# soldasim/BOSS.jl

Hardware: AMD Instinct MI355X
Metric: gp_posterior_updates_per_sec (+ acq_evals_per_sec), N=4096 d=8 fp64 (higher is better)
Workload: dtype f64; 1 GPU; d=8 synthetic blackbox, GaussianProcess(Matern52) surrogate, N=4096 fp64 posterior update + ExpectedImprovement over 8192 candidates per GPU (BASELINE.json configs[1]+[2]); N=4096, d=8, M_per_gpu=8192, kernel=matern52, parallelism=single GPU: no exchange

## Files before the change

### boss.jl_amd/csrc/bosship.hip

```cpp
#include "../../include/bosship.h"

#include <hip/hip_runtime.h>

#include <algorithm>
#include <cmath>
#include <cstdint>
#include <cstdio>
#include <cstdlib>
#include <atomic>
#include <chrono>
#include <cstring>
#include <functional>
#include <limits>
#include <map>
#include <mutex>
#include <string>
#include <thread>
#include <vector>

#include "gp_kernels.hpp"
#include "potrf.hpp"
#include "chain.hpp"
#include "small_calls.hpp"
#include "rider.hpp"
// ... 225 lines not shown
        HIPCHK(hipEventCreateWithFlags(&c->llg_join[i], hipEventDisableTiming));
    }
    c->lookahead = !(getenv("BOSS_NO_LOOKAHEAD") && atoi(getenv("BOSS_NO_LOOKAHEAD")));
    {
        auto set_nonzero = [](const char* name) {
            const char* v = getenv(name);
            return v && *v && std::strcmp(v, "0") != 0;
        };
        static const bool gate_off = set_nonzero("BOSS_NO_GATE") || set_nonzero("ROCPROF_COUNTER_COLLECTION") || getenv("ROCPROF_COUNTERS") ||
                                     getenv("ROCPROF_COUNTER_GROUPS") || set_nonzero("ROCPROF_ADVANCED_THREAD_TRACE") ||
                                     getenv("ROCPROF_ATT_PARAM_SERIALIZE_ALL") || getenv("ROCP_METRICS") || set_nonzero("AMD_SERIALIZE_KERNEL");
        if (!gate_off) {
            if (set_nonzero("BOSS_DEBUG_WATCH")) {
                unsigned long long* hp = nullptr;
                HIPCHK(hipHostMalloc((void**)&hp, SIG_WORDS * sizeof(unsigned long long), hipHostMallocMapped));
                std::memset(hp, 0, SIG_WORDS * sizeof(unsigned long long));
                HIPCHK(hipHostGetDevicePointer((void**)&c->sig_panel, hp, 0));
                c->sig_panel_host = hp;
#ifdef BOSS_DEBUG_WATCH_BUILD
                HIPCHK(hipMemcpyToSymbol(HIP_SYMBOL(boss::g_dbg), &c->sig_panel, sizeof(void*)));
#endif
                std::thread([hp]() {
                    unsigned long long last[SIG_WORDS] = {0};
                    for (;;) {
                        std::this_thread::sleep_for(std::chrono::milliseconds(500));
                        unsigned long long now[SIG_WORDS];
                        for (int i = 0; i < SIG_WORDS; ++i) now[i] = ((volatile unsigned long long*)hp)[i];
                        if (std::memcmp(now, last, sizeof now) == 0) continue;
                        std::memcpy(last, now, sizeof now);
                        std::fprintf(stderr, "[bosship watch] up %llu wdone %llu panel %llu crit %llu | gate %llu near %llu bulk %llu | strips",
                                     now[SIGW_UP], now[SIGW_WDONE], now[SIGW_PANEL], now[SIGW_CRIT], now[SIGW_GATE], now[SIGW_NEAR], now[SIGW_BULK]);
                        for (int q = 0; q < 8; ++q) std::fprintf(stderr, " %llu", now[SIGW_PROG + SIGW_PROG_STRIDE * q]);
                        std::fprintf(stderr, " | give-ups: first %llu n %llu last %llu; waits ended by mark %llu, by clock %llu", now[SIGW_DBG], now[SIGW_DBG + 1],
                                     now[SIGW_DBG + 2], now[SIGW_DBG + 4], now[SIGW_DBG + 5]);
                        std::fprintf(stderr, "\n");
                    }
                }).detach();
            } else {
                HIPCHK(hipMalloc((void**)&c->sig_panel, SIG_WORDS * sizeof(unsigned long long)));
                HIPCHK(hipMemset(c->sig_panel, 0, SIG_WORDS * sizeof(unsigned long long)));
            }
        }
        c->chain_ok = !gate_off && !set_nonzero("BOSS_NO_CHAIN") && !set_nonzero("HIP_LAUNCH_BLOCKING");
        c->test_drop_chain = set_nonzero("BOSS_TEST_DROP_CHAIN");
        if (c->chain_ok) {
            int* okw = nullptr;
            HIPCHK(hipMalloc((void**)&okw, 4 * sizeof(int)));
            HIPCHK(hipMemset(okw, 0, 4 * sizeof(int)));
            hipStream_t probed[4] = {c->own_stream, c->side_stream, c->chain_stream, c->strip_stream};
            for (int i = 0; i < 4; ++i)
                hipLaunchKernelGGL(chain_probe_wait_kernel, dim3(1), dim3(64), 0, probed[i], c->sig_panel + SIGW_NEAR + 1, 4ull, okw + i);
            int okh[4] = {0, 0, 0, 0};
            bool fine = hipDeviceSynchronize() == hipSuccess && hipMemcpy(okh, okw, sizeof okh, hipMemcpyDeviceToHost) == hipSuccess;
            (void)hipFree(okw);
            if (!(fine && okh[0] && okh[1] && okh[2] && okh[3])) c->chain_ok = false;
            if (getenv("BOSS_CHAIN_VERBOSE"))
                std::fprintf(stderr, "[bosship] resident chain: %s (main / side / chain / strip streams side by side: %d %d %d %d)\n",
                             c->chain_ok ? "on" : "off", okh[0], okh[1], okh[2], okh[3]);
        }
    }
    HIPCHK(hipHostMalloc(&c->pinned, PINNED_BYTES, hipHostMallocDefault));
    std::memset(c->pinned, 0, PINNED_UP_OFF);
    HIPCHK(hipFuncSetAttribute((const void*)potrf_diag_kernel, hipFuncAttributeMaxDynamicSharedMemorySize, DIAG_LDS_BYTES));
    HIPCHK(hipFuncSetAttribute((const void*)potrf_chain_kernel, hipFuncAttributeMaxDynamicSharedMemorySize, CHAIN_LDS_BYTES));
    HIPCHK(hipFuncSetAttribute((const void*)potrf_strips_kernel, hipFuncAttributeMaxDynamicSharedMemorySize, STRIPS_LDS_BYTES));
    {
        int cus = 0;
        if (hipDeviceGetAttribute(&cus, hipDeviceAttributeMultiprocessorCount, c->device) != hipSuccess) cus = 0;
        if (cus > 0) c->n_cus = cus;
    }
    HIPCHK(hipFuncSetAttribute((const void*)small_fit_kernel, hipFuncAttributeMaxDynamicSharedMemorySize, SMALL_LDS_BYTES));
    HIPCHK(hipFuncSetAttribute((const void*)small_llgrad_kernel, hipFuncAttributeMaxDynamicSharedMemorySize, SMALL_LLG_LDS_BYTES));
    HIPCHK(hipFuncSetAttribute((const void*)small_fit_batch_kernel, hipFuncAttributeMaxDynamicSharedMemorySize, SMALL_LDS_BYTES));
    HIPCHK(hipFuncSetAttribute((const void*)small_predict_grad_kernel<true>, hipFuncAttributeMaxDynamicSharedMemorySize, SPG_LDS_BYTES));
    HIPCHK(hipFuncSetAttribute((const void*)small_predict_grad_kernel<false>, hipFuncAttributeMaxDynamicSharedMemorySize, SPG_LDS_BYTES));
    HIPCHK(hipFuncSetAttribute((const void*)potrf_syrk_kernel<2, true>, hipFuncAttributeMaxDynamicSharedMemorySize, 96 * 1024));
    HIPCHK(hipFuncSetAttribute((const void*)rider_step_kernel, hipFuncAttributeMaxDynamicSharedMemorySize, 96 * 1024));
    HIPCHK(hipFuncSetAttribute((const void*)predict_kernel<PredG32>, hipFuncAttributeMaxDynamicSharedMemorySize,
                               PredictLds<PredG32>::BYTES));
    HIPCHK(hipFuncSetAttribute((const void*)prune_head_kernel<PredG32>, hipFuncAttributeMaxDynamicSharedMemorySize,
                               PredictLds<PredG32>::BYTES));
    HIPCHK(hipFuncSetAttribute((const void*)predict_kernel_set<PredG32>, hipFuncAttributeMaxDynamicSharedMemorySize,
                               PredictLds<PredG32>::BYTES));
    HIPCHK(hipFuncSetAttribute((const void*)grad_accum_kernel, hipFuncAttributeMaxDynamicSharedMemorySize, 150 * 1024));
    HIPCHK(hipFuncSetAttribute((const void*)winv_gemv_kernel<1>, hipFuncAttributeMaxDynamicSharedMemorySize, 150 * 1024));
    HIPCHK(hipFuncSetAttribute((const void*)winv_gemv_kernel<2>, hipFuncAttributeMaxDynamicSharedMemorySize, 150 * 1024));
    HIPCHK(hipFuncSetAttribute((const void*)winv_gemv_kernel<4>, hipFuncAttributeMaxDynamicSharedMemorySize, 150 * 1024));
    HIPCHK(hipFuncSetAttribute((const void*)winv_args_kernel<1>, hipFuncAttributeMaxDynamicSharedMemorySize, 150 * 1024));
    HIPCHK(hipFuncSetAttribute((const void*)winv_args_kernel<2>, hipFuncAttributeMaxDynamicSharedMemorySize, 150 * 1024));
    HIPCHK(hipFuncSetAttribute((const void*)winv_args_kernel<4>, hipFuncAttributeMaxDynamicSharedMemorySize, 150 * 1024));
    HIPCHK(hipFuncSetAttribute((const void*)winv_args_kernel<1, true>, hipFuncAttributeMaxDynamicSharedMemorySize, 150 * 1024));
    HIPCHK(hipFuncSetAttribute((const void*)few_back_finish_kernel<PredG32>, hipFuncAttributeMaxDynamicSharedMemorySize,
                               PredictLds<PredG32>::BYTES));
    HIPCHK(hipFuncSetAttribute((const void*)few_w_kernel<PredG32>, hipFuncAttributeMaxDynamicSharedMemorySize, PredictLds<PredG32>::BYTES));
    HIPCHK(hipFuncSetAttribute((const void*)few_finish_kernel<PredG32>, hipFuncAttributeMaxDynamicSharedMemorySize,
                               PredictLds<PredG32>::BYTES));
    HIPCHK(hipFuncSetAttribute((const void*)linvt_kernel<PredG32>, hipFuncAttributeMaxDynamicSharedMemorySize,
                               PredictLds<PredG32>::BYTES));
    HIPCHK(hipFuncSetAttribute((const void*)backsolve_kernel<PredG32>, hipFuncAttributeMaxDynamicSharedMemorySize,
                               PredictLds<PredG32>::BYTES));
    HIPCHK(hipFuncSetAttribute((const void*)backsolve_set_kernel<PredG32>, hipFuncAttributeMaxDynamicSharedMemorySize,
                               PredictLds<PredG32>::BYTES));
    HIPCHK(hipFuncSetAttribute((const void*)grad_accum_set_kernel, hipFuncAttributeMaxDynamicSharedMemorySize, 150 * 1024));
    HIPCHK(hipFuncSetAttribute((const void*)predict_kernel<PredG64>, hipFuncAttributeMaxDynamicSharedMemorySize,
                               PredictLds<PredG64>::BYTES));
    HIPCHK(hipFuncSetAttribute((const void*)predict_kernel<PredG32, true>, hipFuncAttributeMaxDynamicSharedMemorySize,
                               PredictLds<PredG32>::BYTES));
    HIPCHK(hipFuncSetAttribute((const void*)predict_kernel<PredG64, true>, hipFuncAttributeMaxDynamicSharedMemorySize,
                               PredictLds<PredG64>::BYTES));
    HIPCHK(hipFuncSetAttribute((const void*)ei_mc_grad_set_kernel, hipFuncAttributeMaxDynamicSharedMemorySize, MC_GRAD_MAX_LDS));
    HIPCHK(hipFuncSetAttribute((const void*)acqp_grad_set_kernel, hipFuncAttributeMaxDynamicSharedMemorySize, ACQP_GRAD_MAX_LDS));
    HIPCHK(hipFuncSetAttribute((const void*)mean_eval_kernel<true>, hipFuncAttributeMaxDynamicSharedMemorySize, MEAN_MAX_LDS));
    HIPCHK(hipFuncSetAttribute((const void*)kprog_llgrad_tile_kernel, hipFuncAttributeMaxDynamicSharedMemorySize, KPROG_GRAD_MAX_LDS));
    HIPCHK(hipFuncSetAttribute((const void*)kprog_grad_accum_kernel, hipFuncAttributeMaxDynamicSharedMemorySize, KPROG_GRAD_MAX_LDS));
    return BOSS_OK;
}

static int virtual_devices() {
    static const int v = getenv("BOSS_VIRTUAL_DEVICES") ? std::max(0, atoi(getenv("BOSS_VIRTUAL_DEVICES"))) : 0;
    return v;
}
static int visible_devices(int* nphys_out = nullptr) {
    int n = 0;
    if (hipGetDeviceCount(&n) != hipSuccess || n <= 0) return 0;
    if (nphys_out) *nphys_out = n;
    return virtual_devices() > 0 ? virtual_devices() : n;
}

static int get_ctx(int device, Ctx** out) {
    std::lock_guard<std::mutex> lk(g_ctx_mtx);
    auto it = g_ctx.find(device);
    if (it != g_ctx.end()) {
        *out = it->second;
        HIPCHK(hipSetDevice(it->second->device));
        return BOSS_OK;
    }
    int nphys = 0;
    const int n = visible_devices(&nphys);
    if (n <= 0) return fail(BOSS_E_NO_DEVICE, "no HIP device visible (bosship has no CPU fallback)");
    if (device < 0 || device >= n) return fail(BOSS_E_INVALID, "device index out of range");
    const int phys = device % nphys;
    HIPCHK(hipSetDevice(phys));
    Ctx* c = new Ctx();
    c->device = phys;
    c->logical = device;
    int rc = ctx_init(c);
    if (rc) {
        ctx_destroy(c);
        return rc;
    }
    g_ctx[device] = c;
    *out = c;
    return BOSS_OK;
}

static int ws_reserve(Workspace& w, size_t bytes) {
    if (w.bytes >= bytes) return BOSS_OK;
    if (w.p) (void)hipFree(w.p);
    w.p = nullptr;
    w.bytes = 0;
    HIPCHK(dev_malloc(&w.p, bytes));
    w.bytes = bytes;
    return BOSS_OK;
}

struct ProfScope {
// ... 20 lines not shown
        hipEvent_t e;
        (void)hipEventCreate(&e);
        return e;
    }
};

struct boss_gpset {
    Ctx* ctx = nullptr;
    std::atomic<int> refs{0};
    void* slab = nullptr;
    void* host_block = nullptr;
    size_t slab_bytes = 0, host_bytes = 0;
};
static bool slab_cache_on() {
    static const bool v = !(getenv("BOSS_SLAB_CACHE") && atoi(getenv("BOSS_SLAB_CACHE")) == 0) &&
                          !poison_alloc();
    return v;
}
static void gpset_release_storage(boss_gpset* st) {
    Ctx* c = st->ctx;
    void *slab = st->slab, *hb = st->host_block;
    if (c && slab_cache_on()) {
        std::lock_guard<std::mutex> lk(c->slab_mtx);
        if (slab && st->slab_bytes > c->slab_cache_bytes) {
            std::swap(slab, c->slab_cache);
            c->slab_cache_bytes = st->slab_bytes;
        }
        if (hb && st->host_bytes > c->hostblk_cache_bytes) {
            std::swap(hb, c->hostblk_cache);
            c->hostblk_cache_bytes = st->host_bytes;
        }
    }
    if (slab) (void)hipFree(slab);
    if (hb) (void)hipHostFree(hb);
    st->slab = st->host_block = nullptr;
}

struct boss_gp {
    Ctx* ctx = nullptr;
    boss_gpset* set = nullptr;
    int kernel = 0, d = 0, N = 0, Np = 0, nblk = 0, ld = 0;
    double *Xraw = nullptr, *Xsc = nullptr, *y = nullptr, *mean = nullptr, *A = nullptr;
    double *LT = nullptr, *DT2 = nullptr, *avec = nullptr;
    bool have_lt = false;
    double *inv16 = nullptr, *Dinv = nullptr, *Dinv2 = nullptr, *hyp = nullptr, *invlam = nullptr, *scal = nullptr;
    int* info = nullptr;
    unsigned char* discrete_dev = nullptr;
    std::vector<unsigned char> discrete;
    double amp2 = 0.0;
    bool has_mean = false, fitted = false, pending = false, have_dinv = false;
    bool dinv_used = false;
    bool dinv_used_prev = false;
    bool gated = false;
    bool chained = false;
    bool fell_back = false;
    int trail_used = -1;
    double* host_res = nullptr;
    double* host_res_dev = nullptr;
    bool par_in_args = false;
    unsigned long long res_seq = 0;
    bool res_polled = false;
    double* host_par = nullptr;
    hipEvent_t par_ev = nullptr;
    unsigned long long epoch = 0;
    unsigned long long factor_gen = 0, dinv0_gen = ~0ull;
    hipEvent_t dinv_ev = nullptr;
    bool dinv_pending = false;
    bool aug = false;
    int npts = 0, ldx = 0, nhead = 0;
    bool gibbs = false;
    double *lamX = nullptr, *ampX = nullptr, *noiseX = nullptr;
    bool kprog = false;
    bool kgrad = false;
    FitProg* kp = nullptr;
    double *Winv = nullptr, *Linv = nullptr;
    double* W2 = nullptr;
    int w2_np = 0;
    unsigned long long w2_gen = ~0ull;
    bool w2_used = false;
    bool have_winv = false;
    int few_calls = 0;
    int append_calls = 0;
    double* prune_a = nullptr;
    int prune_a_np = 0;
    unsigned long long prune_a_gen = ~0ull;
    int prune_skip = 0, prune_backoff = 0;
    int append_path = 0;
};

struct boss_cand {
    Ctx* ctx = nullptr;
    int d = 0, M = 0, Mp = 0;
    double* Craw = nullptr;
};

struct boss_track {
    Ctx* ctx = nullptr;
    boss_gp* gp = nullptr;
    int d = 0, M = 0, Mp = 0, tiles = 0, Ncap = 0, N = 0;
    unsigned long long epoch = 0;
    double *V = nullptr, *Csc = nullptr, *mu = nullptr, *var = nullptr, *mean = nullptr;
    bool has_mean = false;
    bool gibbs = false;
    double *Clam = nullptr, *Camp = nullptr;
    bool aug = false;
};

static inline int round_up(int x, int m) { return (x + m - 1) / m * m; }
struct SetBatch {
    int nb = 1;
    size_t sA = 0, sInv16 = 0, sDinv = 0, sDinv2 = 0, sW = 0, sX = 0;
    size_t sPar = 0;
};
struct MeanFold {
    const double* J = nullptr;
    size_t sJ = 0;
    int T = 0;
    double* dmean = nullptr;
    double* dtheta = nullptr;
};
static void linv_enqueue(boss_gp* g, hipStream_t s, double* U, double* Lw, const SetBatch& B = SetBatch());
constexpr int MAX_ROWS = 46080;

extern "C" const char* boss_version(void) { return "bosship 0.1.0 (gfx950, fp64 MFMA)"; }
extern "C" const char* boss_last_error(void) { return g_last_error.c_str(); }

extern "C" int boss_device_count(int* n_out) {
    const int n = visible_devices();
    hipError_t e = n > 0 ? hipSuccess : hipErrorNoDevice;
    if (e != hipSuccess || n <= 0) {
        if (n_out) *n_out = 0;
        return fail(BOSS_E_NO_DEVICE, "no HIP device visible (bosship has no CPU fallback)");
    }
    if (n_out) *n_out = n;
    return BOSS_OK;
}

extern "C" int boss_set_stream(int device, void* hip_stream) {
    Ctx* c;
    int rc = get_ctx(device, &c);
    if (rc) return rc;
    std::lock_guard<std::mutex> lk(c->mtx);
    HIPCHK(hipStreamSynchronize(c->stream));
    c->stream = hip_stream ? (hipStream_t)hip_stream : c->own_stream;
    return BOSS_OK;
}

extern "C" int boss_device_sync(int device) {
    Ctx* c;
    int rc = get_ctx(device, &c);
    if (rc) return rc;
    HIPCHK(hipStreamSynchronize(c->stream));
    return BOSS_OK;
}

static bool few_done_ensure(Ctx* c, hipStream_t s) {
    if (c->few_done) return true;
    if (hipMalloc((void**)&c->few_done, sizeof(unsigned long long)) != hipSuccess) {
        (void)hipGetLastError();
        c->few_done = nullptr;
        return false;
    }
    (void)hipMemsetAsync(c->few_done, 0, sizeof(unsigned long long), s);
    c->few_done_cnt = 0;
    return true;
}
// ... 194 lines not shown
```

### boss.jl_amd/csrc/host_factor.inc

```


struct LaunchStamps {
    static constexpr int CAP = 512;
    int n = 0;
    int tag[CAP];
    std::chrono::steady_clock::time_point t[CAP];
    void reset() { n = 0; }
    void add(int what) {
        if (n < CAP) {
            tag[n] = what;
            t[n++] = std::chrono::steady_clock::now();
        }
    }
};
static std::atomic<int> g_stamps_on{-1};
static std::atomic<long long> g_stall_us{2500};
static std::mutex g_stall_mtx;
static std::string g_stall_log;
static bool launch_stamps_on() {
    int v = g_stamps_on.load(std::memory_order_relaxed);
    if (v < 0) {
        v = (getenv("BOSS_LAUNCH_STAMPS") && atoi(getenv("BOSS_LAUNCH_STAMPS"))) ? 1 : 0;
        if (getenv("BOSS_STALL_MS")) g_stall_us.store((long long)(atof(getenv("BOSS_STALL_MS")) * 1000.0));
        g_stamps_on.store(v);
// ... 394 lines not shown
        if (m == 0) {
            if (step_hook && chain_inline) (*step_hook)(k);
            break;
        }
        if (la && (m <= small_m + 1 || chain)) {
            const bool poll = last_rest >= 0 && last_rest == tail_join && bulk_pub != 0;
            if (last_rest >= 0 && !poll) (void)hipStreamWaitEvent(s, c->ev_rest[last_rest], 0);
            last_rest = -1;
            if (chain_inline && plan->tab) {
                const int* off = plan->tab_off;
                hipLaunchKernelGGL(potrf_colupd_tab_kernel, dim3(off[k + 1] - off[k]), dim3(256), 0, s, A, ld, plan->tab + off[k], k, critw);
            } else
                hipLaunchKernelGGL(potrf_colupd_kernel, dim3(2 * m * (m + 1) + m, 1, batch), dim3(256), 0, s, A, ld, bstride, k,
                                   m, m, 0, 1, poll ? c->sig_panel + bulk_pub_word : (unsigned long long*)nullptr, bulk_pub, info, chain ? 1 : 0, -1, critw, budget);
            BOSS_STAMP(2000 + k);
            if (step_hook && chain_inline) (*step_hook)(k);
            continue;
        }
        if (!la) {
            ProfScope ps(c, "potrf_syrk");
            hipLaunchKernelGGL(potrf_syrk_kernel<1>, dim3(m * (m + 1) / 2 + m, 1, batch), dim3(256), 0, s, A, ld, bstride, k,
                               k + 1, m, 0);
            continue;
        }
        {
            const bool poll = last_rest >= 0 && last_rest == tail_join && bulk_pub != 0;
            if (last_rest >= 0 && !poll) (void)hipStreamWaitEvent(s, c->ev_rest[last_rest], 0);
            hipLaunchKernelGGL(potrf_colupd_kernel, dim3(4 * m + 1, 1, batch), dim3(256), 0, s, A, ld, bstride, k, m, 1, 0, 1,
                               poll ? c->sig_panel + bulk_pub_word : (unsigned long long*)nullptr, bulk_pub, info, 0, -1, (unsigned long long*)nullptr, budget);
        }
        last_rest = -1;
#ifdef BOSS_EXPERIMENTS
        static const int exp_norest = getenv("BOSS_EXP_NOREST") ? atoi(getenv("BOSS_EXP_NOREST")) : 0;
#else
        constexpr int exp_norest = 0;
#endif
        if (m >= 2 && exp_norest != 1) {
            const int m2 = m - 1;
            (void)hipEventRecord(c->ev_panel[k], s);
            (void)hipStreamWaitEvent(c->side_stream, c->ev_panel[k], 0);
            if (exp_norest != 2)
                hipLaunchKernelGGL(potrf_syrk_kernel<1>, dim3(m2 * (m2 + 1) / 2 + m2, 1, batch), dim3(256), 0, c->side_stream, A,
                                   ld, bstride, k, k + 2, m2, 0);
            (void)hipEventRecord(c->ev_rest[k], c->side_stream);
            last_rest = k;
        }
    }
    if (la && last_rest >= 0) (void)hipStreamWaitEvent(s, c->ev_rest[last_rest], 0);
}

static void gram_enqueue(Ctx* c, const double* Xsc, size_t xs_bstride, int d, int N, int Np, int kern,
                         const double* hyp, double* A, int ld, size_t bstride, int batch) {
    ProfScope ps(c, "gram");
    const int nt = Np / 64;
    hipLaunchKernelGGL(gram_kernel, dim3(nt * (nt + 1) / 2, 1, batch), dim3(256), 0, c->stream, Xsc, xs_bstride, d, N,
                       Np, kern, hyp, A, ld, bstride, 0);
}

static void gp_release(boss_gp* g) {
    if (!g) return;
    if (g->ctx) (void)hipSetDevice(g->ctx->device);
    if (g->ctx) chain_quiesce(g->ctx);
    if (g->set) {
        if (g->ctx) (void)hipStreamSynchronize(g->ctx->stream);
        if (g->dinv_pending && g->ctx) (void)hipStreamSynchronize(g->ctx->side_stream);
        boss_gpset* st = g->set;
        if (st->refs.fetch_sub(1) == 1) {
            gpset_release_storage(st);
            delete st;
        }
        g->Xraw = g->Xsc = g->y = g->mean = g->A = g->inv16 = g->Dinv = g->Dinv2 = g->invlam = g->scal = nullptr;
        g->lamX = g->ampX = g->noiseX = nullptr;
        g->host_res = g->host_par = nullptr;
        g->set = nullptr;
    }
    void* ptrs[] = {g->Xraw, g->Xsc, g->y, g->mean, g->A, g->inv16, g->Dinv, g->Dinv2, g->LT, g->DT2, g->avec, g->invlam, g->scal, g->discrete_dev};
    for (void* p : ptrs)
        if (p) (void)hipFree(p);
    if (g->host_res) (void)hipHostFree(g->host_res);
    if (g->Winv) (void)hipFree(g->Winv);
    if (g->Linv) (void)hipFree(g->Linv);
    if (g->W2) (void)hipFree(g->W2);
    if (g->prune_a) (void)hipFree(g->prune_a);
    if (g->lamX) (void)hipFree(g->lamX);
    if (g->ampX) (void)hipFree(g->ampX);
    if (g->noiseX) (void)hipFree(g->noiseX);
    if (g->host_par) (void)hipHostFree(g->host_par);
    delete g->kp;
    if (g->par_ev) (void)hipEventDestroy(g->par_ev);
    if (g->dinv_ev) (void)hipEventDestroy(g->dinv_ev);
    delete g;
}

static void pack_points(std::vector<double>& dst, const double* X, int d, int n, int ldp,
                        const unsigned char* discrete) {
    dst.assign((size_t)d * ldp, 0.0);
    for (int j = 0; j < n; ++j)
        for (int k = 0; k < d; ++k) {
            double v = X[(size_t)j * d + k];
            if (discrete && discrete[k]) v = std::nearbyint(v);
            dst[(size_t)k * ldp + j] = v;
        }
}

static int gp_create_common(int device, int kernel, int d, int npts, int N, const double* X, const double* y,
                            const unsigned char* discrete, bool aug, boss_gp_t** out) {
    if (!out) return fail(BOSS_E_INVALID, "out is NULL");
    *out = nullptr;
    if (kernel < 0 || kernel > 2) return fail(BOSS_E_INVALID, "unknown kernel id");
    if (d < 1 || N < 1 || !X || !y) return fail(BOSS_E_INVALID, "need d >= 1, N >= 1 and non-NULL X, y");
    if (N > MAX_ROWS) return fail(BOSS_E_INVALID, "more than 46080 rows (observations, or n (1 + d) with gradients) are not supported");
    Ctx* c;
    int rc = get_ctx(device, &c);
    if (rc) return rc;
    boss_gp* g = new boss_gp();
    g->ctx = c;
    g->kernel = kernel;
    g->d = d;
    g->N = N;
    g->Np = round_up(N, PRED_RB);
    g->nblk = g->Np / BLK;
    g->ld = g->Np + RHS_ROWS;
    g->aug = aug;
    g->npts = npts;
    g->nhead = npts;
    g->ldx = aug ? round_up(npts, 64) : g->Np;
    const size_t Np = g->Np, ldx = g->ldx;
#define GALLOC(ptr, bytes)                                        \
    do {                                                          \
        hipError_t e_ = dev_malloc((void**)&(ptr), (bytes));       \
        if (e_ != hipSuccess) {                                   \
            gp_release(g);                                        \
            return fail(BOSS_E_ALLOC, "device allocation failed"); \
        }                                                         \
    } while (0)
    GALLOC(g->Xraw, sizeof(double) * d * ldx);
    GALLOC(g->Xsc, sizeof(double) * d * ldx);
    GALLOC(g->y, sizeof(double) * Np);
    GALLOC(g->mean, sizeof(double) * Np);
    GALLOC(g->A, sizeof(double) * (size_t)g->ld * Np);
    GALLOC(g->inv16, sizeof(double) * g->nblk * 8 * 256);
    GALLOC(g->Dinv, sizeof(double) * g->nblk * BLK * BLK);
    GALLOC(g->Dinv2, sizeof(double) * (g->Np / PRED_RB) * PRED_RB * PRED_RB);
    GALLOC(g->invlam, sizeof(double) * (d + 4));
    g->hyp = g->invlam + d;
    GALLOC(g->scal, sizeof(double) * 4);
    g->info = (int*)(g->scal + 2);
    if (hipHostMalloc((void**)&g->host_res, 512, hipHostMallocDefault) != hipSuccess ||
        hipHostMalloc((void**)&g->host_par, sizeof(double) * (d + 4), hipHostMallocDefault) != hipSuccess ||
        hipEventCreateWithFlags(&g->par_ev, hipEventDisableTiming) != hipSuccess ||
        hipEventCreateWithFlags(&g->dinv_ev, hipEventDisableTiming) != hipSuccess ||
        hipHostGetDevicePointer((void**)&g->host_res_dev, g->host_res, 0) != hipSuccess) {
        gp_release(g);
        return fail(BOSS_E_ALLOC, "pinned allocation failed");
    }
    std::memset(g->host_res, 0, 512);
    if (discrete) {
        g->discrete.assign(discrete, discrete + d);
        bool any = false;
        for (int k = 0; k < d; ++k) any |= discrete[k] != 0;
        if (any) {
            GALLOC(g->discrete_dev, d);
            (void)hipMemcpy(g->discrete_dev, discrete, d, hipMemcpyHostToDevice);
        } else {
            g->discrete.clear();
        }
// ... 559 lines not shown
```

### boss.jl_amd/csrc/host_prune.inc

```

struct PruneCfg {
    int min_tiles = -1;
    int K = 64;
    int s = 1;
    int cap = 1024;
    double slack = 1.0;
};
static PruneCfg g_prune;
constexpr double PRUNE_KMU = 1.2e-4, PRUNE_KVAR = 1e-10;
constexpr size_t PRUNE_RES_OFF = 16;

static bool prune_enabled() {
    static const bool on = !(getenv("BOSS_ACQ_PRUNE") && atoi(getenv("BOSS_ACQ_PRUNE")) == 0);
    static const bool once = [] {
        if (getenv("BOSS_ACQ_PRUNE_BLOCKS")) g_prune.s = std::max(1, atoi(getenv("BOSS_ACQ_PRUNE_BLOCKS")));
        if (getenv("BOSS_ACQ_PRUNE_CAP")) g_prune.cap = std::max(0, atoi(getenv("BOSS_ACQ_PRUNE_CAP")));
        return true;
    }();
    (void)once;
    return on;
}

extern "C" int boss_debug_acq_path(int device, int* out) {
    if (!out) return fail(BOSS_E_INVALID, "out is NULL");
// ... 1 lines not shown
    int rc = get_ctx(device, &c);
    if (rc) return rc;
    std::lock_guard<std::mutex> lk(c->mtx);
    for (int i = 0; i < 5; ++i) out[i] = c->prune_last[i];
    return BOSS_OK;
}
extern "C" int boss_debug_acq_prune_set(int device, int min_tiles, int K, int s, int cap) {
    (void)device;
    (void)prune_enabled();
    const PruneCfg def;
    if (min_tiles != -1) g_prune.min_tiles = min_tiles < -1 ? def.min_tiles : min_tiles;
    if (K != -1) g_prune.K = K < 1 ? def.K : K;
    if (s != -1) g_prune.s = s < 1 ? def.s : s;
    if (cap != -1) g_prune.cap = cap < -1 ? def.cap : cap;
    return BOSS_OK;
}
extern "C" int boss_debug_acq_counters(const boss_gp* g, long* out) {
    if (!g || !out) return fail(BOSS_E_INVALID, "NULL argument");
    out[0] = g->have_winv ? 1 : 0;
    out[1] = g->few_calls;
    out[2] = g_dev_allocs.load();
    out[3] = g->ctx->prune_launches;
    return BOSS_OK;
}
extern "C" int boss_debug_acq_prune_slack(int device, double scale) {
    (void)device;
    if (!(scale >= 0.0)) return fail(BOSS_E_INVALID, "scale must be >= 0");
    g_prune.slack = scale;
    return BOSS_OK;
}
extern "C" int boss_debug_acq_prune_bounds(int device, int M, double* mua_out, double* vars_out, double* ub_out) {
    Ctx* c;
    int rc = get_ctx(device, &c);
    if (rc) return rc;
    std::lock_guard<std::mutex> lk(c->mtx);
    if (M < 1 || M != c->prune_M || !c->prunews.p) return fail(BOSS_E_INVALID, "no pruned attempt with that many candidates");
    HIPCHK(hipStreamSynchronize(c->stream));
    const double* base = (const double*)c->prunews.p;
    if (mua_out) HIPCHK(hipMemcpy(mua_out, base, sizeof(double) * M, hipMemcpyDeviceToHost));
    if (vars_out) HIPCHK(hipMemcpy(vars_out, base + M, sizeof(double) * M, hipMemcpyDeviceToHost));
    if (ub_out) HIPCHK(hipMemcpy(ub_out, base + 2 * (size_t)M, sizeof(double) * M, hipMemcpyDeviceToHost));
    return BOSS_OK;
}

static bool prune_eligible(const boss_gp* g, const boss_cand* cd, int P, int S, const EiPar& par, bool has_out, bool defer, bool has_mc,
                           const double* dpair) {
    if (!prune_enabled() || has_out || defer || dpair || has_mc || P != 1 || S != 1 || par.mode != 1) return false;
    if (g->aug || g->gibbs || g->kprog || g->ctx->prof_on) return false;
    const int ftiles = (cd->M + 31) / 32;
    const int min_tiles = g_prune.min_tiles >= 0 ? g_prune.min_tiles : few_max_tiles();
    if (few_off() || ftiles <= min_tiles || g->Np < 4 * PRED_RB || g->d > 64 || cd->d != g->d || slab_bn(cd->M, false) != 32) return false;
    if (small_predict_ok(g, cd->M) || cd->M <= g_prune.K || cd->M > PRUNE_THREADS * PRUNE_CPT_MAX) return false;
    if (g_prune.K > 32 * few_max_tiles()) return false;
    return g_prune.s < g->Np / PRED_RB;
}

static bool prune_poll(Ctx* c, hipStream_t s, const double* res, unsigned long long want) {
    volatile const unsigned long long* seq = reinterpret_cast<volatile const unsigned long long*>(res) + 4;
    bool got = false;
    for (unsigned long i = 1;; ++i) {
        if (*seq == want) {
            got = true;
            break;
        }
        if ((i & 0x3fff) == 0 && hipStreamQuery(s) != hipErrorNotReady) break;
    }
    std::atomic_thread_fence(std::memory_order_acquire);
    if (!got) {
        (void)hipStreamSynchronize(s);
        got = *seq == want;
    }
    return got;
}

static int prune_avec(boss_gp* g, hipStream_t s, const double** a_out, bool* rebuilt) {
    *rebuilt = false;
    if (g->have_lt && g->avec) {
        *a_out = g->avec;
        return BOSS_OK;
    }
    if (g->prune_a && g->prune_a_np != g->Np) {
        (void)hipStreamSynchronize(s);
        (void)hipFree(g->prune_a);
        g->prune_a = nullptr;
    }
    if (!g->prune_a) {
        if (dev_malloc((void**)&g->prune_a, sizeof(double) * 2 * (size_t)g->Np) != hipSuccess) {
            g->prune_a = nullptr;
            return fail(BOSS_E_ALLOC, "device allocation failed");
        }
        g->prune_a_np = g->Np;
        g->prune_a_gen = ~0ull;
    }
    if (g->prune_a_gen != g->factor_gen) {
        const int nb = g->Np / PRED_RB;
        for (int ib = nb - 1; ib >= 0; --ib)
            hipLaunchKernelGGL(prune_avec_step_kernel, dim3(std::max(1, 2 * ib)), dim3(PRUNE_AVEC_THREADS), 0, s, (const double*)g->A, g->ld, g->Np, g->N,
                               (const double*)g->Dinv2, ib, ib == nb - 1 ? 1 : 0, g->prune_a + g->Np, g->prune_a);
        g->prune_a_gen = g->factor_gen;
        *rebuilt = true;
    }
    *a_out = g->prune_a;
    return BOSS_OK;
}

static int acq_prune_try(boss_gp* g, const boss_cand* cd, const double* mean_dev, const unsigned char* mask_dev, const EiPar& par,
                         bool* done, double* res_out, long* idx_out) {
    *done = false;
    Ctx* c = g->ctx;
    hipStream_t s = c->stream;
    int* last = c->prune_last;
    last[0] = 0;
    last[1] = last[2] = last[4] = 0;
    last[3] = g_prune.s;
    if (g->prune_skip > 0) {
        --g->prune_skip;
        last[0] = 3;
        return BOSS_OK;
    }
    const int M = cd->M, Mp = cd->Mp, d = g->d, Np = g->Np, nch = Np / PRUNE_MU_ROWS, sblk = g_prune.s, K = g_prune.K;
    const int cap = std::min(g_prune.cap, 32 * few_max_tiles()), tiles = (M + 31) / 32;
    const size_t nint = (size_t)round_up(std::max(K, cap), 64);
    const size_t nd = (size_t)4 * M + (size_t)nch * M + 3 * nint + (size_t)d * nint + 2;
    int rc = ws_reserve(c->prunews, sizeof(double) * nd + sizeof(int) * (nint + (size_t)M) + (size_t)M);
    if (rc) return rc;
    rc = ws_reserve(c->csc, sizeof(double) * (size_t)d * Mp);
    if (rc) return rc;
    rc = ws_reserve(c->vscratch, sizeof(double) * (size_t)tiles * 32 * Np);
    if (rc) return rc;
    double* mua = (double*)c->prunews.p;
    double* vars = mua + M;
    double* ub = vars + M;
    unsigned long long* keys = (unsigned long long*)(ub + M);
    double* part = ub + 2 * (size_t)M;
    double* imu = part + (size_t)nch * M;
    double* ivar = imu + nint;
    double* imean = ivar + nint;
    double* icraw = imean + nint;
    double* tpair = icraw + (size_t)d * nint;
    int* sel = (int*)(tpair + 2);
    int* surv = sel + nint;
    unsigned char* insel = (unsigned char*)(surv + M);
    c->prune_M = M;
    double* res = (double*)c->pinned + PRUNE_RES_OFF;

    if (!g->have_dinv) {
        dinv_join(g);
        dinv_launch(g, s);
        g->have_dinv = true;
    }
    dinv_join(g);
    g->dinv_used = true;
    const double* avec = nullptr;
    bool rebuilt = false;
    rc = prune_avec(g, s, &avec, &rebuilt);
    if (rc) return rc;
    last[4] = rebuilt ? 1 : 0;
    c->prune_launches += (rebuilt ? Np / PRED_RB : 0) + 7;
    double* Csc = (double*)c->csc.p;
    hipLaunchKernelGGL(scale_cand_kernel, dim3((Mp + 255) / 256), dim3(256), 0, s, cd->Craw, Csc, g->invlam, g->discrete_dev, d, Mp);
    typedef PredG32 G;
    hipLaunchKernelGGL(prune_head_kernel<G>, dim3(tiles), dim3(G::NTHREADS), PredictLds<G>::BYTES, s, (const double*)g->A, g->ld, Np, g->N,
                       (const double*)g->Dinv2, (const double*)g->Xsc, (const double*)Csc, d, Mp, g->kernel, g->amp2, (double*)c->vscratch.p, M,
                       sblk, vars);
    const size_t mu_lds = sizeof(double) * ((size_t)d + 1) * PRUNE_MU_STAGE;
    auto mu_fn = d <= 16 ? prune_mu_kernel<true> : prune_mu_kernel<false>;
    hipLaunchKernelGGL(mu_fn, dim3((M + PRUNE_MU_CANDS - 1) / PRUNE_MU_CANDS, nch), dim3(256), mu_lds, s, (const double*)g->Xsc, Np, g->N, (const double*)Csc, d, Mp, M,
                       g->kernel, g->amp2, avec, part);
    PrunePar pp;
    pp.coef = par.coefs[0];
    pp.best = par.best;
    pp.amp2 = g->amp2;
    pp.kmu = PRUNE_KMU * g_prune.slack;
    pp.kvar = PRUNE_KVAR * g_prune.slack;
    hipLaunchKernelGGL(prune_bound_kernel, dim3((M + 255) / 256), dim3(256), 0, s, (const double*)part, nch, mean_dev, (const double*)vars, mask_dev, M,
                       pp, mua, ub, keys);
    hipLaunchKernelGGL(prune_select_kernel, dim3(1), dim3(PRUNE_THREADS), 0, s, (const unsigned long long*)keys, M, K, sel, insel);

    boss_cand icd;
    icd.ctx = c;
    icd.d = d;
// ... 45 lines not shown
```

### boss.jl_amd/csrc/prune_kernels.hpp

```cpp
#pragma once
#include "acq_kernels.hpp"

namespace boss {

template <int NC>
__device__ __forceinline__ void prune_wave_sums(double (&v)[NC], int lane) {
#pragma unroll
    for (int h = NC / 2; h >= 1; h >>= 1) {
        const bool up = (lane & h) != 0;
#pragma unroll
        for (int j = 0; j < h; ++j) {
            const double keep = up ? v[j + h] : v[j], send = up ? v[j] : v[j + h];
            v[j] = keep + __shfl_xor(send, h);
        }
    }
#pragma unroll
    for (int off = NC; off < 64; off <<= 1) v[0] += __shfl_xor(v[0], off);
}
constexpr int PRUNE_AVEC_THREADS = 1024;
__global__ __launch_bounds__(PRUNE_AVEC_THREADS) void prune_avec_step_kernel(const double* __restrict__ A, int ld, int Np, int N,
                                                                             const double* __restrict__ Dinv2, int ib, int first,
                                                                             double* __restrict__ r, double* __restrict__ a) {
    __shared__ double rv[PRED_RB], av[PRED_RB];
    const int tid = threadIdx.x, lane = tid & 63;
    const int wave = __builtin_amdgcn_readfirstlane(tid >> 6);
    const int i0 = ib * PRED_RB;
    if (tid < PRED_RB) {
        const int i = i0 + tid;
        rv[tid] = first ? (i < N ? A[(size_t)i * ld + Np] : 0.0) : r[i];
    }
    __syncthreads();
    const double* D = Dinv2 + (size_t)ib * PRED_RB * PRED_RB;
    double r4[4];
#pragma unroll
    for (int q = 0; q < 4; ++q) r4[q] = rv[lane + 64 * q];
    {
        double sums[16];
#pragma unroll
        for (int j = 0; j < 16; ++j) {
            const int c = 16 * j + wave;
            const double* col = D + (size_t)c * PRED_RB;
            double sacc = 0.0;
#pragma unroll
            for (int q = 0; q < 4; ++q) {
                if (q >= j / 4) {
                    const int row = lane + 64 * q;
                    const double dv = col[row];
                    sacc = __builtin_fma(row >= c ? dv : 0.0, r4[q], sacc);
                }
            }
            sums[j] = sacc;
        }
        prune_wave_sums<16>(sums, lane);
        if (lane < 16) av[16 * lane + wave] = sums[0];
    }
    __syncthreads();
    if (blockIdx.x == 0 && tid < PRED_RB) a[i0 + tid] = av[tid];
    if (ib == 0) return;
    double a4[4];
#pragma unroll
    for (int q = 0; q < 4; ++q) a4[q] = av[lane + 64 * q];
    double sums[8];
    const int cg0 = blockIdx.x * 128 + wave * 8;
#pragma unroll
    for (int j = 0; j < 8; ++j) {
        const double* col = A + (size_t)(cg0 + j) * ld + i0;
        double sacc = 0.0;
#pragma unroll
        for (int q = 0; q < 4; ++q) sacc = __builtin_fma(col[lane + 64 * q], a4[q], sacc);
        sums[j] = sacc;
    }
    prune_wave_sums<8>(sums, lane);
    if (lane < 8) {
        const int cg = cg0 + lane;
        const double base = first ? (cg < N ? A[(size_t)cg * ld + Np] : 0.0) : r[cg];
        r[cg] = base - sums[0];
    }
}

template <class G>
__global__ __launch_bounds__(G::NTHREADS) __attribute__((amdgpu_waves_per_eu(1, 1))) void prune_head_kernel(
    const double* __restrict__ A, int ld, int Np, int N, const double* __restrict__ Dinv, const double* __restrict__ Xsc,
    const double* __restrict__ Csc, int d, int Mp, int kern, double amp2, double* __restrict__ Vscratch, int M, int sblk,
    double* __restrict__ var_out) {
    static_assert(G::WC == 1 && G::BM == 2 * BLK && G::PM == 2 && G::WR == 4, "written for the 256-row, 32-candidate geometry");
    constexpr int RB = G::BM;
    extern __shared__ double lds[];
    constexpr int BN = G::BN, TM = G::TM, TN = G::TN, LDR = PredictLds<G>::LDR;
    double* Rs = lds;
    double* red = Rs + RB * LDR;
    const int tid = threadIdx.x, lane = tid & 63;
    const int wave = __builtin_amdgcn_readfirstlane(tid >> 6);
    const int wr = wave, wc = 0;
    const int tile = blockIdx.x, c0 = tile * BN;
    double* V = Vscratch + (size_t)tile * sblk * RB * BN;
    double* part = red + 2 * G::WR * G::BN;
#pragma unroll
    for (int u = 0; u < TN * 4; ++u) part[u * G::NTHREADS + tid] = 0.0;
    double* cs = part + (size_t)G::NTHREADS * PredictLds<G>::PART;
    const bool cs_ok = d <= PRED_CS_MAX_D;
    if (cs_ok) {
        for (int idx = tid; idx < d * BN; idx += G::NTHREADS) cs[idx] = Csc[(size_t)(idx / BN) * Mp + c0 + (idx % BN)];
        __syncthreads();
    }
    for (int ib = 0; ib < sblk; ++ib) {
        v4d acc[TM][TN];
#pragma unroll
        for (int m = 0; m < TM; ++m)
#pragma unroll
            for (int n = 0; n < TN; ++n) acc[m][n] = v4d{0.0, 0.0, 0.0, 0.0};
        G::template run<1>(A + (size_t)ib * RB, ld, V, BN, ib * RB, acc);
        double r2[TM][TN][4];
#pragma unroll
        for (int m = 0; m < TM; ++m)
#pragma unroll
            for (int n = 0; n < TN; ++n)
#pragma unroll
                for (int i = 0; i < 4; ++i) r2[m][n][i] = 0.0;
        if (cs_ok) {
            for (int kd0 = 0; kd0 < d; kd0 += 4) {
                double xr[4][TM];
#pragma unroll
                for (int kk = 0; kk < 4; ++kk)
#pragma unroll
                    for (int m = 0; m < TM; ++m)
                        xr[kk][m] = (kd0 + kk < d) ? Xsc[(size_t)(kd0 + kk) * Np + ib * RB + G::row_of(wr, m, lane)] : 0.0;
#pragma unroll
                for (int kk = 0; kk < 4; ++kk) {
                    if (kd0 + kk < d) {
#pragma unroll
                        for (int n = 0; n < TN; ++n)
#pragma unroll
                            for (int i = 0; i < 4; ++i) {
                                const double xc = cs[(kd0 + kk) * BN + G::col_of(wc, n, i, lane)];
#pragma unroll
                                for (int m = 0; m < TM; ++m) {
                                    const double diff = xr[kk][m] - xc;
                                    r2[m][n][i] = __builtin_fma(diff, diff, r2[m][n][i]);
                                }
                            }
                    }
                }
            }
        } else
        for (int kd = 0; kd < d; ++kd) {
            double xr[TM], xc[TN][4];
#pragma unroll
            for (int m = 0; m < TM; ++m) xr[m] = Xsc[(size_t)kd * Np + ib * RB + G::row_of(wr, m, lane)];
#pragma unroll
            for (int n = 0; n < TN; ++n)
#pragma unroll
                for (int i = 0; i < 4; ++i) xc[n][i] = Csc[(size_t)kd * Mp + c0 + G::col_of(wc, n, i, lane)];
#pragma unroll
            for (int m = 0; m < TM; ++m)
#pragma unroll
                for (int n = 0; n < TN; ++n)
#pragma unroll
                    for (int i = 0; i < 4; ++i) {
// ... 409 lines not shown
```

Before: 913.8 updates/s.

## Restructure prune a-vector solve to precompute off-diagonal products and shorten critical chain

The blocked back-substitution that builds the prune a-vector now starts with one launch that uses a tiled GEMM routine to precompute Y blocks (the product of the next row-block of A with the triangular Dinv2 block). Each step folds the next block's contribution through Y directly into the a computation, so the r update is deferred by one block and its dependency is removed from the serial chain. Thread count drops to 512 and work is spread over more, smaller workgroups. This costs extra scratch memory and an up-front GEMM, and the indexing in the new recurrence is easy to get wrong.

```diff
diff --git a/boss.jl_amd/csrc/bosship.hip b/boss.jl_amd/csrc/bosship.hip
--- a/boss.jl_amd/csrc/bosship.hip
+++ b/boss.jl_amd/csrc/bosship.hip
@@ -331,6 +331,8 @@
                                PredictLds<PredG32>::BYTES));
     HIPCHK(hipFuncSetAttribute((const void*)predict_kernel_set<PredG32>, hipFuncAttributeMaxDynamicSharedMemorySize,
                                PredictLds<PredG32>::BYTES));
+    HIPCHK(hipFuncSetAttribute((const void*)prune_avec_step_kernel<PredG32, true>, hipFuncAttributeMaxDynamicSharedMemorySize,
+                               PruneYLds<PredG32>::BYTES));
     HIPCHK(hipFuncSetAttribute((const void*)grad_accum_kernel, hipFuncAttributeMaxDynamicSharedMemorySize, 150 * 1024));
     HIPCHK(hipFuncSetAttribute((const void*)winv_gemv_kernel<1>, hipFuncAttributeMaxDynamicSharedMemorySize, 150 * 1024));
     HIPCHK(hipFuncSetAttribute((const void*)winv_gemv_kernel<2>, hipFuncAttributeMaxDynamicSharedMemorySize, 150 * 1024));
@@ -517,6 +519,7 @@
     int few_calls = 0;
     int append_calls = 0;
     double* prune_a = nullptr;
+    double* prune_y = nullptr;
     int prune_a_np = 0;
     unsigned long long prune_a_gen = ~0ull;
     int prune_skip = 0, prune_backoff = 0;
diff --git a/boss.jl_amd/csrc/host_factor.inc b/boss.jl_amd/csrc/host_factor.inc
--- a/boss.jl_amd/csrc/host_factor.inc
+++ b/boss.jl_amd/csrc/host_factor.inc
@@ -500,6 +500,7 @@
     if (g->Linv) (void)hipFree(g->Linv);
     if (g->W2) (void)hipFree(g->W2);
     if (g->prune_a) (void)hipFree(g->prune_a);
+    if (g->prune_y) (void)hipFree(g->prune_y);
     if (g->lamX) (void)hipFree(g->lamX);
     if (g->ampX) (void)hipFree(g->ampX);
     if (g->noiseX) (void)hipFree(g->noiseX);
diff --git a/boss.jl_amd/csrc/host_prune.inc b/boss.jl_amd/csrc/host_prune.inc
--- a/boss.jl_amd/csrc/host_prune.inc
+++ b/boss.jl_amd/csrc/host_prune.inc
@@ -107,21 +107,31 @@
     if (g->prune_a && g->prune_a_np != g->Np) {
         (void)hipStreamSynchronize(s);
         (void)hipFree(g->prune_a);
-        g->prune_a = nullptr;
+        if (g->prune_y) (void)hipFree(g->prune_y);
+        g->prune_a = g->prune_y = nullptr;
     }
     if (!g->prune_a) {
+        const int nb = g->Np / PRED_RB;
         if (dev_malloc((void**)&g->prune_a, sizeof(double) * 2 * (size_t)g->Np) != hipSuccess) {
             g->prune_a = nullptr;
             return fail(BOSS_E_ALLOC, "device allocation failed");
         }
+        if (dev_malloc((void**)&g->prune_y, sizeof(double) * (size_t)nb * PRUNE_Y_SLAB) != hipSuccess) {
+            (void)hipFree(g->prune_a);
+            g->prune_a = g->prune_y = nullptr;
+            return fail(BOSS_E_ALLOC, "device allocation failed");
+        }
         g->prune_a_np = g->Np;
         g->prune_a_gen = ~0ull;
     }
     if (g->prune_a_gen != g->factor_gen) {
+        typedef PredG32 G;
         const int nb = g->Np / PRED_RB;
-        for (int ib = nb - 1; ib >= 0; --ib)
-            hipLaunchKernelGGL(prune_avec_step_kernel, dim3(std::max(1, 2 * ib)), dim3(PRUNE_AVEC_THREADS), 0, s, (const double*)g->A, g->ld, g->Np, g->N,
-                               (const double*)g->Dinv2, ib, ib == nb - 1 ? 1 : 0, g->prune_a + g->Np, g->prune_a);
+        hipLaunchKernelGGL((prune_avec_step_kernel<G, true>), dim3(PRUNE_AVEC_PA + 8 * (nb - 1)), dim3(PRUNE_AVEC_THREADS), PruneYLds<G>::BYTES, s,
+                           (const double*)g->A, g->ld, g->Np, g->N, (const double*)g->Dinv2, g->prune_y, nb, nb - 1, g->prune_a + g->Np, g->prune_a);
+        for (int ib = nb - 2; ib >= 0; --ib)
+            hipLaunchKernelGGL((prune_avec_step_kernel<G, false>), dim3(PRUNE_AVEC_PA + 8 * ib), dim3(PRUNE_AVEC_THREADS), 0, s, (const double*)g->A, g->ld,
+                               g->Np, g->N, (const double*)g->Dinv2, g->prune_y, nb, ib, g->prune_a + g->Np, g->prune_a);
         g->prune_a_gen = g->factor_gen;
         *rebuilt = true;
     }
diff --git a/boss.jl_amd/csrc/prune_kernels.hpp b/boss.jl_amd/csrc/prune_kernels.hpp
--- a/boss.jl_amd/csrc/prune_kernels.hpp
+++ b/boss.jl_amd/csrc/prune_kernels.hpp
@@ -17,63 +17,123 @@
 #pragma unroll
     for (int off = NC; off < 64; off <<= 1) v[0] += __shfl_xor(v[0], off);
 }
-constexpr int PRUNE_AVEC_THREADS = 1024;
+constexpr int PRUNE_AVEC_THREADS = 512;
+constexpr int PRUNE_AVEC_PA = 16;
+constexpr int PRUNE_AVEC_BCOLS = 32;
+constexpr size_t PRUNE_Y_SLAB = (size_t)PRED_RB * PRED_RB;
+template <class G>
+struct PruneYLds {
+    static constexpr int LDR = G::BN + 16;
+    static constexpr int BYTES = PRED_RB * LDR * 8;
+};
+
+template <class G>
+__device__ __forceinline__ void prune_y_body(const double* __restrict__ A, int ld, const double* __restrict__ Dinv2,
+                                             double* __restrict__ Y, int i, int c0, double* __restrict__ Rs) {
+    constexpr int RB = G::BM, TM = G::TM, TN = G::TN, LDR = PruneYLds<G>::LDR;
+    static_assert(RB == PRED_RB && G::BN == 32 && TN == 2 && TM % 2 == 0 && G::WC == 1 && G::NTHREADS <= PRUNE_AVEC_THREADS,
+                  "256-row blocks, 32 columns per workgroup");
+    const int tid = threadIdx.x, lane = tid & 63;
+    const int wave = __builtin_amdgcn_readfirstlane(tid >> 6);
+    const double* D = Dinv2 + (size_t)i * RB * RB + (size_t)c0 * RB;
+#pragma unroll 8
+    for (int t = 0; t < RB * 32 / PRUNE_AVEC_THREADS; ++t) {
+        const int idx = tid + PRUNE_AVEC_THREADS * t, k = idx % RB, q = idx / RB;
+        const double dv = D[idx];
+        Rs[k * LDR + q] = k >= c0 + q ? dv : 0.0;
+    }
+    __syncthreads();
+    if (wave >= G::NWAVES) return;
+    v4d acc[TM][TN];
+#pragma unroll
+    for (int m = 0; m < TM; ++m)
+#pragma unroll
+        for (int n = 0; n < TN; ++n) acc[m][n] = v4d{0.0, 0.0, 0.0, 0.0};
+    G::run_Blds(A + (size_t)(i + 1) * RB + (size_t)(i * RB + c0) * ld, ld, Rs + c0 * LDR, LDR, RB - c0, acc);
+    double* Yb = Y + (size_t)i * PRUNE_Y_SLAB;
+#pragma unroll
+    for (int m = 0; m < TM; m += 2) {
+        const int row = G::row_of(wave, m, lane);
+#pragma unroll
+        for (int n = 0; n < TN; ++n)
+#pragma unroll
+            for (int u = 0; u < 4; ++u)
+                *reinterpret_cast<v2d*>(Yb + row + (size_t)(c0 + G::col_of(0, n, u, lane)) * RB) = v2d{acc[m][n][u], acc[m + 1][n][u]};
+    }
+}
+
+template <class G, bool YB>
 __global__ __launch_bounds__(PRUNE_AVEC_THREADS) void prune_avec_step_kernel(const double* __restrict__ A, int ld, int Np, int N,
-                                                                             const double* __restrict__ Dinv2, int ib, int first,
-                                                                             double* __restrict__ r, double* __restrict__ a) {
-    __shared__ double rv[PRED_RB], av[PRED_RB];
+                                                                             const double* __restrict__ Dinv2, double* Y, int nb,
+                                                                             int ib, double* r, double* a) {
     const int tid = threadIdx.x, lane = tid & 63;
     const int wave = __builtin_amdgcn_readfirstlane(tid >> 6);
     const int i0 = ib * PRED_RB;
-    if (tid < PRED_RB) {
-        const int i = i0 + tid;
-        rv[tid] = first ? (i < N ? A[(size_t)i * ld + Np] : 0.0) : r[i];
-    }
-    __syncthreads();
-    const double* D = Dinv2 + (size_t)ib * PRED_RB * PRED_RB;
-    double r4[4];
-#pragma unroll
-    for (int q = 0; q < 4; ++q) r4[q] = rv[lane + 64 * q];
-    {
-        double sums[16];
-#pragma unroll
-        for (int j = 0; j < 16; ++j) {
-            const int c = 16 * j + wave;
-            const double* col = D + (size_t)c * PRED_RB;
+    const bool has_next = ib <= nb - 2;
+    if ((int)blockIdx.x < PRUNE_AVEC_PA) {
+        const bool from_z = ib >= nb - 2;
+        double r4[4], n4[4];
+#pragma unroll
+        for (int q = 0; q < 4; ++q) {
+            const int row = i0 + lane + 64 * q;
+            r4[q] = from_z ? (row < N ? A[(size_t)row * ld + Np] : 0.0) : r[row];
+            n4[q] = has_next ? a[row + PRED_RB] : 0.0;
+        }
+        const int c0 = 16 * (int)blockIdx.x + 2 * wave;
+        const double* D = Dinv2 + (size_t)ib * PRED_RB * PRED_RB + (size_t)c0 * PRED_RB;
+        const double* Yc = Y + (size_t)ib * PRUNE_Y_SLAB + (size_t)c0 * PRED_RB;
+        double dv[2][4], yv[2][4];
+#pragma unroll
+        for (int j = 0; j < 2; ++j)
+#pragma unroll
+            for (int q = 0; q < 4; ++q) {
+                dv[j][q] = D[j * PRED_RB + lane + 64 * q];
+                yv[j][q] = has_next ? Yc[j * PRED_RB + lane + 64 * q] : 0.0;
+            }
+        double sums[2];
+#pragma unroll
+        for (int j = 0; j < 2; ++j) {
             double sacc = 0.0;
 #pragma unroll
-            for (int q = 0; q < 4; ++q) {
-                if (q >= j / 4) {
-                    const int row = lane + 64 * q;
-                    const double dv = col[row];
-                    sacc = __builtin_fma(row >= c ? dv : 0.0, r4[q], sacc);
-                }
-            }
+            for (int q = 0; q < 4; ++q) sacc = __builtin_fma(lane + 64 * q >= c0 + j ? dv[j][q] : 0.0, r4[q], sacc);
+#pragma unroll
+            for (int q = 0; q < 4; ++q) sacc = __builtin_fma(-yv[j][q], n4[q], sacc);
             sums[j] = sacc;
         }
-        prune_wave_sums<16>(sums, lane);
-        if (lane < 16) av[16 * lane + wave] = sums[0];
-    }
-    __syncthreads();
-    if (blockIdx.x == 0 && tid < PRED_RB) a[i0 + tid] = av[tid];
-    if (ib == 0) return;
-    double a4[4];
-#pragma unroll
-    for (int q = 0; q < 4; ++q) a4[q] = av[lane + 64 * q];
-    double sums[8];
-    const int cg0 = blockIdx.x * 128 + wave * 8;
-#pragma unroll
-    for (int j = 0; j < 8; ++j) {
-        const double* col = A + (size_t)(cg0 + j) * ld + i0;
+        prune_wave_sums<2>(sums, lane);
+        if (lane < 2) {
+            const int row = i0 + c0 + lane;
+            a[row] = row < N ? sums[0] : 0.0;
+        }
+        return;
+    }
+    const int n = (int)blockIdx.x - PRUNE_AVEC_PA;
+    if (YB) {
+        extern __shared__ double lds[];
+        prune_y_body<G>(A, ld, Dinv2, Y, n >> 3, 32 * (n & 7), lds);
+        return;
+    }
+    const int s0 = i0 + PRED_RB;
+    const int cg0 = n * PRUNE_AVEC_BCOLS + wave * 4;
+    double a4[4], lv[4][4];
+#pragma unroll
+    for (int q = 0; q < 4; ++q) a4[q] = a[s0 + lane + 64 * q];
+#pragma unroll
+    for (int j = 0; j < 4; ++j)
+#pragma unroll
+        for (int q = 0; q < 4; ++q) lv[j][q] = A[(size_t)(cg0 + j) * ld + s0 + lane + 64 * q];
+    double sums[4];
+#pragma unroll
+    for (int j = 0; j < 4; ++j) {
         double sacc = 0.0;
 #pragma unroll
-        for (int q = 0; q < 4; ++q) sacc = __builtin_fma(col[lane + 64 * q], a4[q], sacc);
+        for (int q = 0; q < 4; ++q) sacc = __builtin_fma(lv[j][q], a4[q], sacc);
         sums[j] = sacc;
     }
-    prune_wave_sums<8>(sums, lane);
-    if (lane < 8) {
+    prune_wave_sums<4>(sums, lane);
+    if (lane < 4) {
         const int cg = cg0 + lane;
-        const double base = first ? (cg < N ? A[(size_t)cg * ld + Np] : 0.0) : r[cg];
+        const double base = ib == nb - 2 ? (cg < N ? A[(size_t)cg * ld + Np] : 0.0) : r[cg];
         r[cg] = base - sums[0];
     }
 }
```

Measured after the change: 911.9 updates/s (median of 2 runs). About the same (-0.2%).
